# sb17v/GaussianK-SGD

Measured on AMD Instinct MI355X. Metric: images/sec (whole node) ResNet-50 k=0.1% at 1/2/4/8 MI355X; effective grad compression ratio, higher is better.
Workload: dtype fp32; 1 GPU; model=resnet50, global_batch=512, per_gpu_batch=512, image_size=224, parallelism=dp1, compressor=gaussian, buckets=1, threshold=524288000, planner=threshold, exchange=local, momentum_correction=True, hip_graph=False, f32_matmul=bf16x6

## Files before the change

### gaussiank_sgd_amd/ops/autotune.py

```python
from __future__ import annotations

import os
from typing import Callable, Dict, Iterable, List, Optional, Tuple

import torch

_TUNE = os.environ.get("GKSGD_GEMM_TUNE", "1") != "0"
_choices: Dict[tuple, tuple] = {}
_OWN = ("hip", "w3", "mat", "wino", "wx6")
_GK_MARGIN = float(os.environ.get("GKSGD_GK_MARGIN", "0.05"))
_timings: Dict[tuple, list] = {}
_NT_CFGS = [1, 2, 3, 4, 11, 13, 21, 22, 23, 24, 111, 113, 121, 122, 123, 124, 25, 26, 27, 125, 126, 127,
            211, 212, 213, 214, 221, 222, 223, 224]
NT_GRIDS = (0, 512, 1 << 20)
_TN_CFGS = [(c, s) for c in (1, 2, 3, 4, 5, 6, 7, 8, 21, 22, 23, 24, 27, 9, 29, 101, 121, 102, 122) for s in (0, 128)]
_NT_CFGS_F32 = [1, 2, 3, 4, 7, 11, 12, 13, 14, 21, 22, 23, 24, 101, 102, 103, 104, 201, 202, 203, 204,
                1001, 1002, 1003, 1004, 1005, 1006, 1007, 1021, 1022, 1101, 1102, 1103]
_TN_CFGS_F32 = [(c, s) for c in (1, 2, 3, 4, 5, 6, 7, 8, 9, 11, 12, 13, 14, 15, 16) for s in (0, 64)]
_TN_SMALL_M = 1 << 17
_TN_SMALL_F32 = [(c, s) for c in (4, 5, 11, 14, 15) for s in (16, 32, 128)]


X6 = 100000
_NT_CFGS_X6 = [c + X6 for c in (1, 2, 3, 4, 5, 6, 7, 12, 13, 101, 102, 103, 104, 105, 106, 107, 202, 203, 1001, 1002, 1003)]
_NT_CFGS_X62 = [2 * X6 + t for t in range(1, 8)] + [3 * X6 + t for t in range(1, 8)]
_F32MM = os.environ.get("GKSGD_F32_MATMUL", "bf16x6")


def set_f32_matmul(mode: str) -> str:
    global _F32MM
    if mode not in ("native", "bf16x6"):
        raise ValueError("f32 matmul mode must be 'native' or 'bf16x6', got %r" % (mode,))
# ... 156 lines not shown
```

### gaussiank_sgd_amd/ops/build.py

```python
from __future__ import annotations

import argparse
import concurrent.futures as cf
import hashlib
import os
import re
import shutil
import subprocess
import sys
import sysconfig
from pathlib import Path
from typing import List

PKG = Path(__file__).resolve().parents[1]
REPO = PKG.parent
CSRC = PKG / "ops" / "csrc"
BUILD = REPO / "build" / "gksgd_ext"
TARGET = PKG / "_C.so"
ASAN = os.environ.get("GKSGD_ASAN", "0") == "1"
if ASAN:
    BUILD = REPO / "build" / "gksgd_ext_asan"
    TARGET = REPO / "build" / "asan" / "_C.so"
SAN_HOST = ["-fsanitize=address", "-fsanitize=undefined"]
VARIANT = os.environ.get("GKSGD_VARIANT", "")
VARIANT_FLAGS = os.environ.get("GKSGD_VARIANT_FLAGS", "").split()
if VARIANT and not ASAN:
    BUILD = REPO / "build" / ("gksgd_ext_" + VARIANT)
    TARGET = REPO / "variants" / VARIANT / "_C.so"
ARCH = os.environ.get("GKSGD_OFFLOAD_ARCH", "gfx950")
ROCM = os.environ.get("ROCM_PATH", "/opt/rocm")

GEMM_UNIT_FAMILY = ["nt", "nt", "nt", "nt", "tn", "nt", "nt", "tn", "nt_x62", "tn_x62", "nt_x62"]
HIP_SOURCES = [
    "kernels/compress.hip",
    "kernels/quality.hip",
    "kernels/scatter.hip",
    "kernels/optim.hip",
    "kernels/bn_act.hip",
    "kernels/gemm.hip",
    *["kernels/gemm_inst_%s.hip#%d" % (f, u) for u, f in enumerate(GEMM_UNIT_FAMILY)],
    "kernels/ln.hip",
    "kernels/linear.hip",
    "kernels/lstm.hip",
    "kernels/stem.hip",
    "kernels/wgrad3.hip",
    "kernels/attn.hip",
    "kernels/attn_f32.hip",
    "kernels/embed.hip",
    "kernels/xent.hip",
    "kernels/winograd.hip",
    "kernels/wino_x6.hip",
    "kernels/stem_f32.hip",
    "kernels/prep.hip",
]
CXX_SOURCES = [
    "comm/rccl_engine.cpp",
    "bindings.cpp",
]
EXTRA_FLAGS = {"kernels/scatter.hip": ["-ffp-contract=off"],
               **{"kernels/gemm_inst_%s.hip" % f: ["-fno-slp-vectorize"] for f in set(GEMM_UNIT_FAMILY)}}


def _torch_dirs():
    import torch
    tdir = Path(torch.__file__).resolve().parent
    return tdir / "include", tdir / "include" / "torch" / "csrc" / "api" / "include", tdir / "lib"


def _hipcc() -> str:
    p = shutil.which("hipcc") or os.path.join(ROCM, "bin", "hipcc")
    return p


def _hip_flags() -> List[str]:
    san = []
    if ASAN:
        for f in SAN_HOST:
            san += ["-Xarch_host", f]
        san += ["-Xarch_host", "-fno-omit-frame-pointer"]
    return san + VARIANT_FLAGS + [
        "--offload-arch=" + ARCH,
        "-O3",
        "-fPIC",
# ... 131 lines not shown
```

### gaussiank_sgd_amd/ops/conv1x1.py

```python
from __future__ import annotations

import os
from itertools import product
from typing import Dict

import torch
import torch.nn as nn
import torch.nn.functional as F

from . import autotune
from . import load
from . import streams
from . import weight_prep
from .autotune import (X6, f32_matmul, load_choices, save_choices, set_f32_matmul,
                       tuned_choices, tuning_log)

_CL = torch.channels_last
_ENABLED = os.environ.get("GKSGD_FASTCONV", "1") != "0"
_BIAS_COLSUM = os.environ.get("GKSGD_CONV_BIAS_COLSUM", "1") != "0"
_WINO = os.environ.get("GKSGD_WINO", "1") != "0"
_FORCE = os.environ.get("GKSGD_CONV_FORCE", "")
_WINO_GRIDS = (0, 1 << 20)
_zeros: Dict[torch.device, torch.Tensor] = {}

# ... 286 lines not shown
    return ch is None or ch[0] == "hip"


def _dgrad_bn_ds(dy: torch.Tensor, w: torch.Tensor, x_shape, link, wp: bool = False) -> torch.Tensor:
    N, C, H, W, K, k, p, OH, OW = _geom(x_shape, w, 1)
    g = _g()
    M = N * H * W
    dt = dy.dtype
    dz = torch.empty(x_shape, dtype=dt, device=dy.device, memory_format=_CL)
    st = torch.empty(2, min(1280, (M + 63) // 64), C, dtype=torch.float32, device=dy.device)
    DY, DZ, H2 = _rows(dy), _rows(dz), _rows(link.h)
    D2, geo, mask = link.dy2c, list(link.geo), link.mask
    Wt = _lazy(lambda: weight_prep.transposed_1x1(w, wp))
    run = lambda c, mb: g.gemm_nt(DY, Wt(), DZ, c, mb, st, None, H2, D2, mask, bn_dy2_geo=geo)
    cands = autotune.hip_cands(run, product(autotune.nt_x62_cfgs(), autotune.NT_GRIDS))
    ch = autotune.pick(("dgrad_bn_ds", N, C, H, W, K) + autotune.dkey(dt), cands)
    rows = run(ch[1], ch[2])
    link.part = (st, int(rows))
    link.dz = dz
    link.dy2c = None
    return dz


def _bn_fusable(link, s: int, dgrad_key: tuple) -> bool:
    if link is None or s != 1 or not _link_on() or not link.ready():
        return False
    if link.h.dtype != dgrad_key_dtype(dgrad_key):
        return False
    ch = autotune.choice(dgrad_key)
    return ch is None or ch[0] in ("hip", "wino", "wx6")


def dgrad_key_dtype(key: tuple) -> torch.dtype:
    return torch.float32 if "f32" in key[8:] else torch.bfloat16


def _wgrad_key(x: torch.Tensor, w: torch.Tensor, s: int, lz=None) -> tuple:
    N, C, H, W, K, k, p, OH, OW = _geom(x.shape, w, s)
    wino = lz is None and _wino_ok(x.dtype, k, s, C, K) and C % 64 == 0 and _wino_shape_fits(N, H, W, C, K)
    return ("wgrad", N, C, H, W, K, k, s) + autotune.dkey(x.dtype) + (("lz",) if lz is not None else ()) + \
        (("wino",) if wino else ())


def _wgrad_into(dy: torch.Tensor, x: torch.Tensor, w: torch.Tensor, s: int, out_f32: torch.Tensor, lz=None,
                plink=None, side: bool = False) -> None:
    N, C, H, W, K, k, p, OH, OW = _geom(x.shape, w, s)
# ... 108 lines not shown
        gvb = getattr(bs0, "grad_view", None) if bs0 is not None else None
        bias_fork = fork and _FORK_BIAS and _BIAS_COLSUM and gvb is not None and gvb.is_contiguous() and \
            not getattr(bs0, "shared", False) and dy.is_contiguous(memory_format=_CL)

        def fork_wgrad():
            sink.check()
            if bias_fork:
                bs0.check()
            side = streams.fork(x.device)
            with torch.cuda.stream(side):
                _wgrad_into(dy, x, w, s, sink.grad_view, side=True)
                if bias_fork:
                    from .linear import bias_grad_acc_
                    bias_grad_acc_(gvb, _rows(dy))
            streams.hold(x.device, dy, x, w)
        if fork and not _WGRAD_AFTER:
            fork_wgrad()
        dx = None
        if ctx.needs_input_grad[0]:
            N, C, H, W = x.shape
            key = _dgrad_key(N, C, H, W, w.shape[0], w.shape[2], s, ctx.dt)
            prep, ctx.prep = ctx.prep, None
            with weight_prep.use(prep):
                if lz is None and _ds_compact_ok(ds_link, x, w, s, ctx.dt):
                    ds_link.dy2c = _dgrad_ds(dy, w, x.shape, wp=ctx.wp)
                    ds_link.geo = (H, W, dy.shape[2], dy.shape[3])
                elif link is not None and link.dy2c is not None:
                    if _ds_fusable(link, x, w, s, ctx.dt, key, lz):
                        dx = _dgrad_bn_ds(dy, w, x.shape, link, wp=ctx.wp)
                    else:
                        dx = _dgrad(dy, w, x.shape, s, lz, plink, wp=ctx.wp)
                elif _bn_fusable(link, s, key):
                    dx = _dgrad_bn(dy, w, x.shape, s, link, lz, plink, wp=ctx.wp)
                else:
                    dx = _dgrad(dy, w, x.shape, s, lz, plink, wp=ctx.wp)
        if fork and _WGRAD_AFTER:
            fork_wgrad()
        gparam = None
        if ctx.needs_input_grad[1] and not fork:
            if direct:
                sink.check()
                _wgrad_into(dy, x, w, s, sink.grad_view, lz, plink)
            else:
                out = torch.zeros(w.shape, dtype=torch.float32, device=x.device).contiguous(memory_format=_CL)
                _wgrad_into(dy, x, w, s, out, lz, plink)
                if sink is not None:
                    sink(out)
# ... 93 lines not shown
```

### gaussiank_sgd_amd/ops/csrc/bindings.cpp

```cpp
#include <ATen/ATen.h>
#include <c10/core/DeviceGuard.h>
#include <c10/hip/HIPStream.h>
#include <torch/custom_class.h>
#include <torch/library.h>

#include <cstring>
#include <vector>

#include "comm/rccl_engine.h"
#include "kernels/gemm_cfg.h"
#include "kernels/gk_kernels.h"

namespace {

hipStream_t cur_stream(const at::Tensor& t) {
  return c10::hip::getCurrentHIPStream(t.device().index()).stream();
}

void check_dev(const at::Tensor& t, const char* name) {
  TORCH_CHECK(t.is_cuda(), name, " must be a GPU tensor");
  TORCH_CHECK(t.is_contiguous(), name, " must be contiguous");
}

void check_f32(const at::Tensor& t, const char* name) {
// ... 1466 lines not shown
  if (k == 1) {
    const at::Tensor wt = w.reshape({K, C}).t().contiguous();
    const int r = gk::conv_nt_remap(dy.data_ptr(), K, zero.data_ptr(), (int)OHd, (int)OWd, (int)K, (int)OHd,
                                    (int)OWd, 1, 1, wt.data_ptr(), dx.data_ptr(), N * OHd * OWd, (int)C, (int)H, (int)W,
                                    0, 0, 1, f32, (int)cfg, (int)max_blocks, lz, st);
    TORCH_CHECK(r >= 0, "conv_dgrad_s2: the lazy operand's coefficient table does not fit this tile configuration");
    return;
  }
  const at::Tensor wt = w.permute({1, 2, 3, 0}).contiguous();
  for (int a = 0; a < 2; ++a) {
    for (int b = 0; b < 2; ++b) {
      const int64_t OHc = (H - a + 1) / 2, OWc = (W - b + 1) / 2;
      if (OHc <= 0 || OWc <= 0) continue;
      at::Tensor wc = a == 0 ? wt.slice(1, 1, 2) : wt.slice(1, 0, 3, 2).flip({1});
      wc = b == 0 ? wc.slice(2, 1, 2) : wc.slice(2, 0, 3, 2).flip({2});
      wc = wc.contiguous();
      const int r = gk::conv_nt_remap(dy.data_ptr(), K, zero.data_ptr(), (int)OHd, (int)OWd, (int)K, (int)OHc,
                                      (int)OWc, a == 0 ? 1 : 2, b == 0 ? 1 : 2, wc.data_ptr(), dx.data_ptr(),
                                      N * OHc * OWc, (int)C, (int)H, (int)W, a, b, 0, f32, (int)cfg, (int)max_blocks,
                                      lz, st);
      TORCH_CHECK(r >= 0, "conv_dgrad_s2: the lazy operand's coefficient table does not fit this tile configuration");
    }
  }
}

int64_t wgrad3_ws(int64_t N, int64_t H, int64_t W, int64_t C, int64_t K) {
  return gk::wgrad3_ws_floats((int)N, (int)H, (int)W, (int)C, (int)K);
}

void conv3_wgrad(at::Tensor dy, at::Tensor x, at::Tensor out, at::Tensor part, at::Tensor zero) {
  TORCH_CHECK(x.is_cuda() && x.scalar_type() == at::kBFloat16 && x.dim() == 4 &&
                  x.is_contiguous(at::MemoryFormat::ChannelsLast),
              "conv3_wgrad: x must be channels-last bf16 [N, C, H, W]");
  const int64_t N = x.size(0), C = x.size(1), H = x.size(2), W = x.size(3);
  TORCH_CHECK(dy.is_cuda() && dy.scalar_type() == at::kBFloat16 && dy.dim() == 4 && dy.size(0) == N &&
                  dy.size(2) == H && dy.size(3) == W && dy.is_contiguous(at::MemoryFormat::ChannelsLast),
              "conv3_wgrad: dy must be channels-last bf16 [N, K, H, W]");
  const int64_t K = dy.size(1);
  TORCH_CHECK(gk::wgrad3_supported((int)H, (int)W, (int)C, (int)K), "conv3_wgrad: unsupported shape");
  TORCH_CHECK(N * H * W < (int64_t(1) << 31), "conv3_wgrad: too many pixels");
  TORCH_CHECK(out.is_cuda() && out.scalar_type() == at::kFloat && out.dim() == 4 && out.size(0) == K &&
                  out.size(1) == C && out.size(2) == 3 && out.size(3) == 3,
              "conv3_wgrad: out must be fp32 [K, C, 3, 3]");
  TORCH_CHECK(part.is_cuda() && part.scalar_type() == at::kFloat && part.is_contiguous() &&
                  part.numel() >= wgrad3_ws(N, H, W, C, K),
              "conv3_wgrad: part must hold wgrad3_ws floats");
// ... 566 lines not shown
  m.def("stem_f32_supported(int H, int W) -> bool", [](int64_t H, int64_t W) { return gk::stem_f32_supported((int)H, (int)W); });
  m.def("stem_f32_fwd(Tensor x, Tensor w, Tensor(a!) y, Tensor(b!)? stats=None) -> int");
  m.def("stem_f32x6_wplanes() -> int", &stem_f32x6_wplanes);
  m.def("stem_f32x6_fwd(Tensor x, Tensor w, Tensor(a!) y, Tensor(b!)? stats, Tensor(c!) wp3) -> int");
  m.def("stem_f32_wgrad_ws(int N) -> int", &stem_f32_wgrad_ws);
  m.def("stem_f32_wgrad(Tensor x, Tensor dy, Tensor(a!) out, Tensor(b!) part, bool x6=False) -> ()");
  m.def("wgrad3_supported(int H, int W, int C, int K) -> bool", [](int64_t H, int64_t W, int64_t C, int64_t K) {
    return gk::wgrad3_supported((int)H, (int)W, (int)C, (int)K);
  });
  m.def("wgrad3_ws(int N, int H, int W, int C, int K) -> int", &wgrad3_ws);
  m.def("conv3_wgrad(Tensor dy, Tensor x, Tensor(a!) out, Tensor(b!) part, Tensor zero) -> ()");
  m.def("wino_weights(Tensor w, Tensor(a!) u, bool flip) -> ()");
  m.def("weight_prep(Tensor table, int ndesc, int total_blocks) -> ()");
  m.def("weight_prep_blocks(int kind, int R, int S) -> int", &weight_prep_blocks);
  m.def("wino_wgrad_ws(int N, int H, int W, int C, int K, int splits=0) -> int", &wino_wgrad_ws);
  m.def("wino_wgrad(Tensor x, Tensor dy, Tensor(a!) out, Tensor(b!) part, int splits=0) -> ()");
  m.def("wino_conv(Tensor x, Tensor u, Tensor(a!) y, int max_blocks=0, Tensor(b!)? stats=None, Tensor? bn_h=None, "
        "Tensor? bn_dy2=None, Tensor? bn_mask=None, int splits=1) -> int");
  m.def("wino_x6_weights(Tensor w, Tensor(a!) u3, bool flip) -> ()");
  m.def("wino_x6_conv(Tensor x, Tensor u3, Tensor(a!) y, int max_blocks=0, Tensor(b!)? stats=None, "
        "Tensor? bn_h=None, Tensor? bn_dy2=None, Tensor? bn_mask=None) -> int");
  m.def("conv_dgrad_s2(Tensor dy, Tensor w, Tensor(a!) dx, Tensor zero, int cfg=0, int max_blocks=0, "
        "Tensor? lz_x=None, Tensor? lz_coef=None, Tensor? lz_padz=None, Tensor? lz_padx=None) -> ()");
  m.def("bn_bwd_lazy_pre(Tensor x, Tensor part, int rows, Tensor? w, Tensor mean, Tensor invstd, "
        "Tensor(a!) dgamma, Tensor(b!) dbeta, Tensor(c!) coef, Tensor(d!) padz, Tensor(e!) padx, "
        "Tensor(f!)? gw_acc=None, Tensor(g!)? gb_acc=None) -> ()");
  m.def("bn_act_backward_lazy(Tensor dy, Tensor? dy2, Tensor? mask, Tensor x, Tensor(a!) dz, Tensor? w, "
        "Tensor mean, Tensor invstd, Tensor(b!) dgamma, Tensor(c!) dbeta, Tensor(d!) ws, bool relu, "
        "Tensor(e!) coef, Tensor(f!) padz, Tensor(g!) padx, Tensor(h!)? gw_acc=None, Tensor(i!)? gb_acc=None) -> ()");
  m.def("bn_lazy_apply(Tensor dz, Tensor x, Tensor(a!) dx, Tensor coef) -> ()");
  m.def("bn_stats_partials(Tensor x, Tensor(a!) ws) -> ()");
  m.def(
      "bn_act_backward_pre_dual(Tensor dz, Tensor x, Tensor(a!) dx, Tensor? w, Tensor mean, Tensor invstd, "
      "Tensor(b!) dgamma, Tensor(c!) dbeta, Tensor part, int rows, Tensor(d!)? gw_acc, Tensor(e!)? gb_acc, Tensor x2, "
      "Tensor(f!) dx2, Tensor? w2, Tensor mean2, Tensor invstd2, Tensor(g!) dgamma2, Tensor(h!) dbeta2, "
      "Tensor(i!) ws2, Tensor(j!)? gw2_acc, Tensor(k!)? gb2_acc) -> ()");
  m.def("bn_act_backward_pre(Tensor dz, Tensor x, Tensor(a!) dx, Tensor? w, Tensor mean, Tensor invstd, "
        "Tensor(b!) dgamma, Tensor(c!) dbeta, Tensor part, int rows, Tensor(d!)? gw_acc=None, "
        "Tensor(e!)? gb_acc=None, Tensor(f!)? fin=None) -> ()");
  m.def("bn_fin_state_bytes(int C) -> int", &bn_fin_state_bytes);
  m.def("attn_supported(int T, int D) -> bool",
        [](int64_t T, int64_t D) { return gk::attn_supported((int)T, (int)D); });
  m.def("attn_fwd(Tensor qkv, Tensor(a!) out, Tensor(b!) lse, int heads, float p, int seed, Tensor? seed_dev=None, "
        "Tensor? key_bits=None, Tensor(c!)? out_lo=None, bool causal=False) -> ()");
  m.def("attn_pack_key_mask(Tensor mask, Tensor(a!) bits) -> ()");
  m.def("attn_bwd(Tensor qkv, Tensor out, Tensor dout, Tensor lse, Tensor(a!) delta, Tensor(b!) dqkv, int heads, "
// ... 70 lines not shown
  m.impl("scatter_add_records", &scatter_add_records);
  m.impl("apply_records_sgd", &apply_records_sgd);
  m.impl("arena_digest", &arena_digest);
  m.impl("fill_zero", &fill_zero);
  m.impl("sign_bucket_compress", &sign_bucket_compress);
  m.impl("sign_bucket_decompress", &sign_bucket_decompress);
  m.impl("fused_sgd", &fused_sgd);
  m.impl("fused_adam", &fused_adam);
  m.impl("fused_lamb", &fused_lamb);
  m.impl("segmented_sumsq", &segmented_sumsq);
  m.impl("fused_lars", &fused_lars);
  m.impl("clip_grad_norm", &clip_grad_norm);
  m.impl("bn_act_forward", &bn_act_forward);
  m.impl("bn_act_finalize", &bn_act_finalize);
  m.impl("bn_act_backward", &bn_act_backward);
  m.impl("bn_act_backward_pre", &bn_act_backward_pre);
  m.impl("bn_act_backward_pre_dual", &bn_act_backward_pre_dual);
  m.impl("bn_bwd_lazy_pre", &bn_bwd_lazy_pre);
  m.impl("bn_act_backward_lazy", &bn_act_backward_lazy);
  m.impl("bn_lazy_apply", &bn_lazy_apply);
  m.impl("bn_stats_partials", &bn_stats_partials);
  m.impl("stem_pack", &stem_pack);
  m.impl("conv_dgrad_s2", &conv_dgrad_s2);
  m.impl("conv3_wgrad", &conv3_wgrad);
  m.impl("stem_fwd", &stem_fwd);
  m.impl("stem_wgrad", &stem_wgrad);
  m.impl("stem_f32_fwd", &stem_f32_fwd);
  m.impl("stem_f32x6_fwd", &stem_f32x6_fwd);
  m.impl("stem_f32_wgrad", &stem_f32_wgrad);
  m.impl("bn_relu_pool_forward", &bn_relu_pool_forward);
  m.impl("bn_relu_pool_backward", &bn_relu_pool_backward);
  m.impl("accum_grad", &accum_grad);
  m.impl("momentum_correct", &momentum_correct);
  m.impl("mask_records", &mask_records);
  m.impl("cast_bf16", &cast_bf16);
  m.impl("gemm_nt", &gemm_nt);
  m.impl("gemm_tn_acc", &gemm_tn_acc);
  m.impl("conv_nt", &conv_nt);
  m.impl("wino_weights", &wino_weights);
  m.impl("weight_prep", &weight_prep);
  m.impl("wino_conv", &wino_conv);
  m.impl("wino_x6_weights", &wino_x6_weights);
  m.impl("wino_x6_conv", &wino_x6_conv);
  m.impl("wino_wgrad", &wino_wgrad);
  m.impl("conv_tn_acc", &conv_tn_acc);
  m.impl("attn_fwd", &attn_fwd);
// ... 19 lines not shown
```

### gaussiank_sgd_amd/ops/csrc/kernels/gemm_nt_x62.h

```cpp
#pragma once

#include "gemm_common.h"

namespace gk {
namespace {

template <int WM, int WN>
struct X62Cfg {
  static constexpr int NW = WM * WN;
  static constexpr int THREADS = 64 * NW;
  static constexpr int BM = 64 * WM;
  static constexpr int BN = 64 * WN;
  static constexpr int PA = BM * 64;
  static constexpr int PB = BN * 64;
  static constexpr int STAGE = 3 * (PA + PB);
  static constexpr int LDS = 2 * STAGE;
  static constexpr int PRA = BM * 4 / THREADS;
  static constexpr int PRB = BN * 4 / THREADS;
  static_assert(PRA >= 1 && PRB >= 1 && (BM * 4) % THREADS == 0 && (BN * 4) % THREADS == 0, "pieces per thread");
  static_assert(LDS <= 160 * 1024, "LDS");
};

template <int WM, int WN, bool BNB, int NPF = 1, bool GATHER = false, bool P3 = false, bool D2C = false>
__global__ void __launch_bounds__(64 * WM * WN) __attribute__((amdgpu_waves_per_eu(1)))
gemm_nt_x62_kernel(const float* __restrict__ A, int64_t lda, const float* __restrict__ B, int64_t ldb,
                   float* __restrict__ C, int64_t ldc, int64_t M, int K, const float* __restrict__ bias,
                   float* __restrict__ stats, int64_t stats_ld, BnBwd bb, ConvGeo geo) {
  using Cfg = X62Cfg<WM, WN>;
  extern __shared__ __attribute__((aligned(16))) char smem[];
  int bx, by;
  xcd_remap2(bx, by);
  const int tid = threadIdx.x;
  const int lane = tid & 63;
  const int wave = __builtin_amdgcn_readfirstlane(tid >> 6);
  const int wm = wave / WN, wn = wave % WN;
  const int fr = lane & 15, fq = lane >> 4;
  const int n0 = by * Cfg::BN;
  const int Ntot = (int)gridDim.y * Cfg::BN;
  const int64_t mtiles = (M + Cfg::BM - 1) / Cfg::BM;
  const int nk = K / 32;
  const int64_t my_tiles = bx < mtiles ? (mtiles - 1 - bx) / gridDim.x + 1 : 0;
  const int T_ = (int)(my_tiles * nk);
  if (T_ == 0) {
    if (stats)
      for (int c = tid; c < Cfg::BN; c += Cfg::THREADS) {
        stats[(int64_t)bx * Ntot + n0 + c] = 0.f;
// ... 137 lines not shown
  for (int a = 0; a < 4; ++a)
#pragma unroll
    for (int b = 0; b < 4; ++b) acc[a][b] = f32x4{0.f, 0.f, 0.f, 0.f};
  float ssum[4][4], ssq[4][4], bia[BNB ? 1 : 4][4];
#pragma unroll
  for (int a = 0; a < 4; ++a)
#pragma unroll
    for (int b = 0; b < 4; ++b) {
      ssum[a][b] = ssq[a][b] = 0.f;
      if constexpr (!BNB) bia[a][b] = bias ? bias[n0 + wn * 64 + a * 16 + fq * 4 + b] : 0.f;
    }

  auto epilogue = [&](int64_t mt) __attribute__((always_inline)) {
    const int64_t mbase = mt * Cfg::BM;
    constexpr int EH = BNB ? 1 : 4;
#pragma unroll
    for (int ms = 0; ms < 4; ++ms) {
      const int64_t m = mbase + wm * 64 + ms * 16 + fr;
      const bool live = m < M;
#pragma unroll
      for (int nh = 0; nh < 4; nh += EH) {
      f32x4 ehv[EH], ed2[EH];
      uint32_t ebits[EH];
      if constexpr (BNB) {
#pragma unroll
        for (int e = 0; e < EH; ++e) {
          ehv[e] = ed2[e] = f32x4{0.f, 0.f, 0.f, 0.f};
          ebits[e] = 0u;
        }
        if (live) {
          int32_t d2row = -1;
          if constexpr (BNB && D2C) {
            const uint32_t mu = (uint32_t)m;
            const uint32_t img = (__umulhi(mu, bb.mg_hw) + mu) >> bb.sh_hw, rem = mu - img * (uint32_t)(bb.H * bb.W);
            const uint32_t ph = (__umulhi(rem, bb.mg_w) + rem) >> bb.sh_w, pw = rem - ph * (uint32_t)bb.W;
            if (((ph | pw) & 1u) == 0u) d2row = (int32_t)((img * (uint32_t)bb.OH + (ph >> 1)) * (uint32_t)bb.OW + (pw >> 1));
          }
#pragma unroll
          for (int e = 0; e < EH; ++e) {
            const int n = n0 + wn * 64 + (nh + e) * 16 + fq * 4;
            ehv[e] = *reinterpret_cast<const f32x4*>(static_cast<const float*>(bb.h) + m * ldc + n);
            if constexpr (D2C) {
              if (d2row >= 0)
                ed2[e] = *reinterpret_cast<const f32x4*>(static_cast<const float*>(bb.dy2) + (int64_t)d2row * ldc + n);
            } else {
              if (bb.dy2) ed2[e] = *reinterpret_cast<const f32x4*>(static_cast<const float*>(bb.dy2) + m * ldc + n);
            }
            ebits[e] = bb.mask ? (uint32_t)bb.mask[m * (Ntot >> 2) + (n >> 2)] : 0xfu;
          }
        }
      }
#pragma unroll
      for (int e = 0; e < EH; ++e) {
        const int ns = nh + e;
        const int n = n0 + wn * 64 + ns * 16 + fq * 4;
        f32x4 v = acc[ms][ns];
        acc[ms][ns] = f32x4{0.f, 0.f, 0.f, 0.f};
        if constexpr (!BNB) {
#pragma unroll
          for (int r = 0; r < 4; ++r) v[r] += bia[ns][r];
        }
        if constexpr (BNB) {
#pragma unroll
          for (int r = 0; r < 4; ++r) {
            const float dz = (ebits[e] >> r) & 1u ? v[r] + ed2[e][r] : 0.f;
            v[r] = dz;
            ssum[ns][r] += dz;
            ssq[ns][r] = fmaf(dz, ehv[e][r], ssq[ns][r]);
          }
        } else {
          if (stats && live) {
#pragma unroll
            for (int r = 0; r < 4; ++r) {
              ssum[ns][r] += v[r];
              ssq[ns][r] = fmaf(v[r], v[r], ssq[ns][r]);
            }
          }
        }
        if (live) *reinterpret_cast<f32x4*>(C + m * ldc + n) = v;
      }
      }
    }
  };

  using I0 = std::integral_constant<int, 0>;
  using I1 = std::integral_constant<int, (NPF > 1 ? 1 : 0)>;
  issue_loads(I0{});
  split_write(0, I0{});
  if (T_ > 1) issue_loads(I1{});
  if (NPF > 1 && T_ > 2) issue_loads(I0{});
  __syncthreads();
  int ks = 0;
  int64_t mt = bx;
  auto slice = [&](int t, auto PAR) __attribute__((always_inline)) {
    constexpr int par = decltype(PAR)::value;
    using SN = std::integral_constant<int, (NPF > 1 ? (par ^ 1) : 0)>;
    const int cur = par;
    const char* st = smem + cur * Cfg::STAGE;
    const char* pa = st;
    const char* pb = st + 3 * Cfg::PA;
    auto frag = [&](const char* plane, int row) __attribute__((always_inline)) -> bf16x8 {
      return *reinterpret_cast<const bf16x8*>(plane + row * 64 + ((fq ^ x62_swz(row)) << 4));
// ... 53 lines not shown
#pragma unroll
      for (int a = 0; a < 4; ++a)
#pragma unroll
        for (int b = 0; b < 4; ++b) {
          const int col = wn * 64 + a * 16 + fq * 4 + b;
          red[wm * Cfg::BN + col] = ssum[a][b];
          red[(WM + wm) * Cfg::BN + col] = ssq[a][b];
        }
    }
    __syncthreads();
    for (int c = tid; c < Cfg::BN; c += Cfg::THREADS) {
      float sa = 0.f, sb = 0.f;
#pragma unroll
      for (int w2 = 0; w2 < WM; ++w2) {
        sa += red[w2 * Cfg::BN + c];
        sb += red[(WM + w2) * Cfg::BN + c];
      }
      stats[(int64_t)bx * Ntot + n0 + c] = sa;
      stats[stats_ld + (int64_t)bx * Ntot + n0 + c] = sb;
    }
  }
}

template <int WM, int WN, bool BNB, int NPF, bool GATHER, bool P3 = false, bool D2C = false>
int launch_nt_x62(const float* A, int64_t lda, const float* B, int64_t ldb, float* C, int64_t ldc, int64_t M, int N,
                  int K, int max_blocks, const float* bias, float* stats, int64_t stats_ld, int stats_rows,
                  const BnBwd& bb, const ConvGeo& geo, hipStream_t stream) {
  using Cfg = X62Cfg<WM, WN>;
  const int ntiles = N / Cfg::BN;
  const int64_t mtiles = (M + Cfg::BM - 1) / Cfg::BM;
  const int per_cu = (160 * 1024) / Cfg::LDS > 0 ? (160 * 1024) / Cfg::LDS : 1;
  int64_t gx = ((int64_t)256 * per_cu + ntiles - 1) / ntiles;
  if (max_blocks > 0) gx = max_blocks;
  if (gx < 1) gx = 1;
  if (gx > mtiles) gx = mtiles;
  if (stats && gx > stats_rows) gx = stats_rows;
  static bool attr = [] {
    return hipFuncSetAttribute(reinterpret_cast<const void*>(&gemm_nt_x62_kernel<WM, WN, BNB, NPF, GATHER, P3, D2C>),
                               hipFuncAttributeMaxDynamicSharedMemorySize, 160 * 1024) == hipSuccess;
  }();
  (void)attr;
  hipLaunchKernelGGL((gemm_nt_x62_kernel<WM, WN, BNB, NPF, GATHER, P3, D2C>), dim3((unsigned)gx, (unsigned)ntiles), dim3(Cfg::THREADS),
                     Cfg::LDS, stream, A, lda, B, ldb, C, ldc, M, K, bias, stats, stats_ld, bb, geo);
  return (int)gx;
}

template <bool GATHER>
int nt_x62_dispatch(const float* A, int64_t lda, const float* B, int64_t ldb, float* C, int64_t ldc, int64_t M,
                    int N, int K, const cfg::NtWord& w, int max_blocks, const float* bias, float* stats,
                    int64_t stats_ld, int stats_rows, const BnBwd& bb, const ConvGeo& geo, hipStream_t stream) {
  const cfg::X62NtSel s = cfg::nt_x62_select(w, N, geo.b3 != nullptr, bb.h != nullptr);
#define GK_X62L(WM_, WN_, BNB_, P3_, D2C_)                                                                   \
  launch_nt_x62<WM_, WN_, BNB_, 1, GATHER, P3_, D2C_>(A, lda, B, ldb, C, ldc, M, N, K, max_blocks, bias, stats, \
                                                      stats_ld, stats_rows, bb, geo, stream)
#define GK_X62N(WM_, WN_, P3_)                                             \
  do {                                                                     \
    if constexpr (!GATHER)                                                 \
      if (s.bnb && bb.OW > 0) return GK_X62L(WM_, WN_, true, P3_, true);   \
    return s.bnb ? GK_X62L(WM_, WN_, true, P3_, false) : GK_X62L(WM_, WN_, false, P3_, false); \
  } while (0)
#define GK_X62(WM_, WN_)               \
  case cfg::x62_key(WM_, WN_):         \
    if (s.p3) GK_X62N(WM_, WN_, true); \
    GK_X62N(WM_, WN_, false)
  switch (cfg::x62_key(s.wm, s.wn)) {
    GK_X62(2, 4);
    GK_X62(4, 2);
    GK_X62(1, 4);
    GK_X62(4, 1);
    GK_X62(1, 2);
    GK_X62(2, 1);
    GK_X62(2, 2);
  }
#undef GK_X62
#undef GK_X62N
#undef GK_X62L
  return cfg::kDoesNotFit;
// ... 5 lines not shown
```

### gaussiank_sgd_amd/ops/csrc/kernels/gk_kernels.h

```cpp
#pragma once

#include <hip/hip_runtime.h>
#include <stddef.h>
#include <stdint.h>

namespace gk {

enum Mode : int {
  kModeGaussian = 0,
  kModeRedSync = 1,
  kModeRedSyncTrim = 2,
  kModeTopK = 3,
  kModeRandomK = 4,
  kModeThreshold = 5,
  kModeDGC = 6,
  kModeGaussianCal = 7,
};

constexpr int kCalFallback = 16;
constexpr int kOverflowExact = 17;

constexpr int kMaxCand = 16;
constexpr int kRecHdr = 4;
constexpr int kMaxCountBlocks = 1024;
// ... 252 lines not shown
};
struct LazyArgs {
  const void* x;
  const float* coef;
  const void* padz;
  const void* padx;
  int C;
};
int gemm_nt(const void* A, int64_t lda, const void* B, int64_t ldb, void* C, int64_t ldc, int64_t M, int N, int K,
            bool f32, int cfg, int max_blocks, float* stats, int stats_rows, const float* bias, const BnBwdArgs* bn,
            const LazyArgs* lazy, hipStream_t stream, float* splitk_ws = nullptr, const void* b3 = nullptr);
int splitk_reduce(const float* ws, int S, int64_t M, int N, float* C, int64_t ldc, const float* bias, float* stats,
                  int stats_rows, const BnBwdArgs* bn, hipStream_t stream);
int gemm_tn_acc(const void* G, int64_t ldg, const void* X, int64_t ldx, float* W, int64_t ldw, int64_t M, int N,
                 int K, bool f32, int cfg, int splits, const LazyArgs* lazy, hipStream_t stream);
int conv_nt(const void* X, const void* zero, int H, int W, int C, int OH, int OW, int S, int P, int KH, int KW,
            const void* B, void* Y, int64_t M, int N, bool f32, int cfg, int max_blocks, float* stats, int stats_rows,
            const float* bias, const BnBwdArgs* bn, const LazyArgs* lazy, hipStream_t stream,
            float* splitk_ws = nullptr, const void* b3 = nullptr);
void split3_rows(const float* src, int64_t ld, void* dst, int64_t R, int S, hipStream_t stream);
int conv_nt_remap(const void* X, int64_t ldx, const void* zero, int H, int W, int C, int OH, int OW, int KH, int KW,
                  const void* B, void* Y, int64_t M, int N, int RH, int RW, int RA, int RB, int RZ, bool f32, int cfg,
                  int max_blocks, const LazyArgs* lazy, hipStream_t stream);
int conv_tn_acc(const void* G, const void* X, const void* zero, int H, int W, int C, int OH, int OW, int S, int P,
                 int KH, int KW, float* Wout, int64_t M, int N, bool f32, int cfg, int splits, const LazyArgs* lazy,
                 hipStream_t stream);
bool stem_f32_supported(int H, int W);
int stem_f32_wgrad_blocks(int N);
int stem_f32x6_wplanes();
int stem_f32x6_forward(const float* x, int N, int H, int W, const float* w, int64_t s0, int64_t s1, int64_t s2,
                       int64_t s3, uint16_t* wp3, float* y, float* stats, int stats_rows, hipStream_t stream);
int stem_f32_forward(const float* x, int N, int H, int W, const float* w, int64_t s0, int64_t s1, int64_t s2,
                     int64_t s3, float* y, float* stats, int stats_rows, hipStream_t stream);
void stem_f32_wgrad(const float* x, const float* dy, int N, int H, int W, float* part, float* out, int64_t s0,
                    int64_t s1, int64_t s2, int64_t s3, bool x6, hipStream_t stream);
void wino_weights(const float* w, float* u, int Co, int Ci, int flip, hipStream_t stream);
enum PrepKind : int32_t { kPrepWino = 0, kPrepWinoFlip = 1, kPrepT32 = 2, kPrepT16 = 3, kPrepWinoX6 = 4,
                          kPrepWinoX6Flip = 5 };
struct PrepDesc {
  const void* src;
  void* dst;
  int64_t ld_in, ld_out;
  int64_t block_begin;
  int32_t kind, R, S, tiles_s;
};
static_assert(sizeof(PrepDesc) == 56, "PrepDesc layout is packed by ops/weight_prep.py");
// ... 95 lines not shown
```

### gaussiank_sgd_amd/ops/weight_prep.py

```python
from __future__ import annotations

import contextlib
import os
import struct
import threading
from typing import Callable, Dict, List, Optional, Tuple

import torch

KIND_WINO, KIND_WINO_FLIP, KIND_T32, KIND_T16, KIND_WINO_X6, KIND_WINO_X6_FLIP = 0, 1, 2, 3, 4, 5
_DESC = struct.Struct("<QQqqqiiii")
_MAX_DESCS = 512
_tls = threading.local()
ENABLED = os.environ.get("GKSGD_WEIGHT_PREP", "1") != "0"


def _ops():
    return torch.ops.gksgd


class _Entry:
    __slots__ = ("src", "dst", "descs", "ready")

    def __init__(self, src: torch.Tensor, dst: torch.Tensor, descs: List[tuple]):
# ... 146 lines not shown


def flipped_3x3(w: torch.Tensor, persistent: bool) -> torch.Tensor:
    K, C = w.shape[0], w.shape[1]

    def make():
        return torch.empty((C, K, 3, 3), dtype=w.dtype, device=w.device, memory_format=torch.channels_last)

    def fill(out):
        out.copy_(w.flip(2, 3).transpose(0, 1))
    p = current()
    if p is None or not persistent or w.dtype not in (torch.float32, torch.bfloat16) or \
            not w.is_contiguous(memory_format=torch.channels_last):
        out = make()
        fill(out)
        return out
    kind = KIND_T32 if w.dtype == torch.float32 else KIND_T16
    es = w.element_size()

    def descs(out):
        return [(kind, w.data_ptr() + (8 - t) * C * es, out.data_ptr() + t * K * es, 9 * C, 9 * K, K, C)
                for t in range(9)]
    return p.acquire(_key("f3", w), w, make, descs, fill)
```

Baseline: 5221 images/s.

## Add bf16x6 stride-2 3x3 dgrad via sub-pixel class decomposition with fused BN backward

Adds a stride-2 3x3 data-gradient path that splits the transposed convolution into four output-parity classes. Each class is a dense implicit GEMM run through the register-staged bf16x6 NT kernel, writing into the strided dx positions through a new S2C epilogue remap. This avoids the zero-stuffed or gather-heavy work of the generic s2 dgrad. An optional fused BN-backward epilogue gathers stats partials in the same pass. The autotuner can still fall back to the existing path, now tagged 'base' and treated as an in-house candidate, at the cost of extra tuning time and a per-call weight reorder when the weights are not persistent.

```diff
diff --git a/gaussiank_sgd_amd/ops/autotune.py b/gaussiank_sgd_amd/ops/autotune.py
--- a/gaussiank_sgd_amd/ops/autotune.py
+++ b/gaussiank_sgd_amd/ops/autotune.py
@@ -7,7 +7,7 @@
 
 _TUNE = os.environ.get("GKSGD_GEMM_TUNE", "1") != "0"
 _choices: Dict[tuple, tuple] = {}
-_OWN = ("hip", "w3", "mat", "wino", "wx6")
+_OWN = ("hip", "w3", "mat", "wino", "wx6", "base")
 _GK_MARGIN = float(os.environ.get("GKSGD_GK_MARGIN", "0.05"))
 _timings: Dict[tuple, list] = {}
 _NT_CFGS = [1, 2, 3, 4, 11, 13, 21, 22, 23, 24, 111, 113, 121, 122, 123, 124, 25, 26, 27, 125, 126, 127,
diff --git a/gaussiank_sgd_amd/ops/build.py b/gaussiank_sgd_amd/ops/build.py
--- a/gaussiank_sgd_amd/ops/build.py
+++ b/gaussiank_sgd_amd/ops/build.py
@@ -38,6 +38,7 @@
     "kernels/optim.hip",
     "kernels/bn_act.hip",
     "kernels/gemm.hip",
+    "kernels/dgrad_s2_x62.hip",
     *["kernels/gemm_inst_%s.hip#%d" % (f, u) for u, f in enumerate(GEMM_UNIT_FAMILY)],
     "kernels/ln.hip",
     "kernels/linear.hip",
@@ -58,7 +59,8 @@
     "bindings.cpp",
 ]
 EXTRA_FLAGS = {"kernels/scatter.hip": ["-ffp-contract=off"],
-               **{"kernels/gemm_inst_%s.hip" % f: ["-fno-slp-vectorize"] for f in set(GEMM_UNIT_FAMILY)}}
+               **{"kernels/gemm_inst_%s.hip" % f: ["-fno-slp-vectorize"] for f in set(GEMM_UNIT_FAMILY)},
+               "kernels/dgrad_s2_x62.hip": ["-fno-slp-vectorize"]}
 
 
 def _torch_dirs():
diff --git a/gaussiank_sgd_amd/ops/conv1x1.py b/gaussiank_sgd_amd/ops/conv1x1.py
--- a/gaussiank_sgd_amd/ops/conv1x1.py
+++ b/gaussiank_sgd_amd/ops/conv1x1.py
@@ -332,6 +332,73 @@
     return dz
 
 
+_S2X = os.environ.get("GKSGD_DGRAD_S2_X62", "1") != "0"
+_BASE = ("base", 0, 0)
+
+
+def _s2x_ok(w: torch.Tensor, s: int, dt: torch.dtype, lz) -> bool:
+    return _S2X and s == 2 and w.shape[2] == 3 and dt == torch.float32 and lz is None and \
+        f32_matmul() == "bf16x6"
+
+
+def _dgrad_s2x(dy: torch.Tensor, w: torch.Tensor, x_shape, wp: bool = False) -> torch.Tensor:
+    N, C, H, W, K, k, p, OH, OW = _geom(x_shape, w, 2)
+    g = _g()
+    dt = dy.dtype
+    dx = torch.empty(x_shape, dtype=dt, device=dy.device, memory_format=_CL)
+    z = _zero(dy.device)
+    wc = _lazy(lambda: weight_prep.s2_class_weights(w, wp))
+    run = lambda c, mb: g.conv_dgrad_s2_x62(dy, wc(), dx, z, c, mb)
+    cands = autotune.hip_cands(run, product(autotune.nt_x62_cfgs(), autotune.NT_GRIDS))
+    cands.append((_BASE, lambda: _dgrad(dy, w, x_shape, 2, wp=wp)))
+    ch = autotune.pick(("dgrad_s2x", N, C, H, W, K) + autotune.dkey(dt), cands)
+    if ch[0] == "base":
+        return _dgrad(dy, w, x_shape, 2, wp=wp)
+    run(ch[1], ch[2])
+    return dx
+
+
+def _dgrad_bn_s2(dy: torch.Tensor, w: torch.Tensor, x_shape, link, wp: bool = False) -> torch.Tensor:
+    N, C, H, W, K, k, p, OH, OW = _geom(x_shape, w, 2)
+    g = _g()
+    dt = dy.dtype
+    dz = torch.empty(x_shape, dtype=dt, device=dy.device, memory_format=_CL)
+    st = torch.empty(2, 4 * min(512, (N * ((H + 1) // 2) * ((W + 1) // 2) + 63) // 64), C, dtype=torch.float32,
+                     device=dy.device)
+    h, mask = link.h, link.mask
+    z = _zero(dy.device)
+    wc = _lazy(lambda: weight_prep.s2_class_weights(w, wp))
+    run = lambda c, mb: g.conv_dgrad_s2_x62(dy, wc(), dz, z, c, mb, st, h, mask)
+    key = ("dgrad_bn", N, C, H, W, K, k, 2, False) + autotune.dkey(dt)
+    cands = autotune.hip_cands(run, product(autotune.nt_x62_cfgs(), autotune.NT_GRIDS))
+    if autotune.choice(key) is None:
+        mean, invstd = torch.zeros(C, device=dy.device), torch.ones(C, device=dy.device)
+        gs = torch.empty(2, C, dtype=torch.float32, device=dy.device)
+        dxs = torch.empty_like(h, memory_format=_CL)
+        ws = torch.empty(int(g.bn_workspace_floats(N * H * W, C, h.element_size())), dtype=torch.float32,
+                         device=dy.device)
+
+        def fused(fn):
+            g.bn_act_backward_pre(dz, h, dxs, None, mean, invstd, gs[0], gs[1], st, int(fn()))
+
+        def base():
+            g.bn_act_backward(_dgrad(dy, w, x_shape, 2, wp=wp), mask, h, dxs, None, None, mean, invstd, gs[0], gs[1],
+                              ws, mask is not None)
+        cands = [(tag, (lambda fn=fn: fused(fn))) for tag, fn in cands] + [(_BASE, base)]
+    ch = autotune.pick(key, cands)
+    if ch[0] == "base":
+        return _dgrad(dy, w, x_shape, 2, wp=wp)
+    rows = run(ch[1], ch[2])
+    link.part = (st, int(rows))
+    link.dz = dz
+    return dz
+
+
+def _bn_s2_fusable(link, x: torch.Tensor, dt: torch.dtype) -> bool:
+    return link is not None and _link_on() and link.ready() and link.dy2 is None and link.dy2c is None and \
+        link.h.dtype == dt and link.h.shape == x.shape
+
+
 def _bn_fusable(link, s: int, dgrad_key: tuple) -> bool:
     if link is None or s != 1 or not _link_on() or not link.ready():
         return False
@@ -486,7 +553,12 @@
             key = _dgrad_key(N, C, H, W, w.shape[0], w.shape[2], s, ctx.dt)
             prep, ctx.prep = ctx.prep, None
             with weight_prep.use(prep):
-                if lz is None and _ds_compact_ok(ds_link, x, w, s, ctx.dt):
+                if _s2x_ok(w, s, ctx.dt, lz):
+                    if _bn_s2_fusable(link, x, ctx.dt):
+                        dx = _dgrad_bn_s2(dy, w, x.shape, link, wp=ctx.wp)
+                    else:
+                        dx = _dgrad_s2x(dy, w, x.shape, wp=ctx.wp)
+                elif lz is None and _ds_compact_ok(ds_link, x, w, s, ctx.dt):
                     ds_link.dy2c = _dgrad_ds(dy, w, x.shape, wp=ctx.wp)
                     ds_link.geo = (H, W, dy.shape[2], dy.shape[3])
                 elif link is not None and link.dy2c is not None:
diff --git a/gaussiank_sgd_amd/ops/csrc/bindings.cpp b/gaussiank_sgd_amd/ops/csrc/bindings.cpp
--- a/gaussiank_sgd_amd/ops/csrc/bindings.cpp
+++ b/gaussiank_sgd_amd/ops/csrc/bindings.cpp
@@ -1512,6 +1512,53 @@
       TORCH_CHECK(r >= 0, "conv_dgrad_s2: the lazy operand's coefficient table does not fit this tile configuration");
     }
   }
+}
+
+int64_t conv_dgrad_s2_x62(at::Tensor dy, at::Tensor wcls, at::Tensor dx, at::Tensor zero, int64_t cfg,
+                          int64_t max_blocks, c10::optional<at::Tensor> stats, c10::optional<at::Tensor> bn_h,
+                          c10::optional<at::Tensor> bn_mask, c10::optional<at::Tensor> lz_x) {
+  TORCH_CHECK(!lz_x.has_value() || !lz_x->defined(), "conv_dgrad_s2_x62: no lazy operand (conv_dgrad_s2 takes one)");
+  TORCH_CHECK(dy.is_cuda() && dy.scalar_type() == at::kFloat && dy.dim() == 4 &&
+                  dy.is_contiguous(at::MemoryFormat::ChannelsLast),
+              "conv_dgrad_s2_x62: dy must be channels-last fp32");
+  TORCH_CHECK(dx.is_cuda() && dx.scalar_type() == at::kFloat && dx.dim() == 4 && dx.size(0) == dy.size(0) &&
+                  dx.is_contiguous(at::MemoryFormat::ChannelsLast),
+              "conv_dgrad_s2_x62: dx must be channels-last fp32 [N, C, H, W]");
+  const int64_t N = dy.size(0), K = dy.size(1), OH = dy.size(2), OW = dy.size(3);
+  const int64_t C = dx.size(1), H = dx.size(2), W = dx.size(3);
+  TORCH_CHECK((H - 1) / 2 + 1 == OH && (W - 1) / 2 + 1 == OW, "conv_dgrad_s2_x62: shape mismatch");
+  TORCH_CHECK(K % 64 == 0 && C % 64 == 0 && dy.numel() > 0, "conv_dgrad_s2_x62: channels must be multiples of 64");
+  TORCH_CHECK(wcls.is_cuda() && wcls.scalar_type() == at::kFloat && wcls.is_contiguous() && wcls.numel() == 9 * C * K &&
+                  reinterpret_cast<uintptr_t>(wcls.data_ptr()) % 16 == 0,
+              "conv_dgrad_s2_x62: wcls must hold the four class matrices, 9 * C * K contiguous fp32");
+  check_zero(zero);
+  TORCH_CHECK(dy.numel() < (int64_t(1) << 31) && N * H * W < (int64_t(1) << 31), "conv_dgrad_s2_x62: too many elements");
+  const gk::cfg::NtWord word = gk::cfg::NtWord::decode((int)cfg);
+  TORCH_CHECK(word.family >= 2 && word.planes <= 1,
+              "conv_dgrad_s2_x62: register-staged bf16x6 configurations only (cfg digit 200000 / 300000)");
+  int rows = 0;
+  float* sp = stats_ptr(stats, C, &rows);
+  gk::BnBwdArgs bn{};
+  const bool has_bn = bn_bwd_args(bn_h, c10::nullopt, bn_mask, N * H * W, C, C, sp != nullptr, at::kFloat, &bn);
+  TORCH_CHECK(!has_bn || rows >= 4, "conv_dgrad_s2_x62: the BN-backward epilogue needs >= 4 partial rows");
+  TORCH_CHECK(has_bn || sp == nullptr, "conv_dgrad_s2_x62: stats come with the BN-backward epilogue only");
+  c10::DeviceGuard guard(dy.device());
+  const hipStream_t st = cur_stream(dy);
+  at::Tensor b3;
+  if (word.family == 3) {
+    b3 = at::empty({27 * C * K}, wcls.options().dtype(at::kBFloat16));
+    for (int cls = 0; cls < 4; ++cls) {
+      const int64_t off = gk::s2_class_offset(cls) * C * K, taps = (1 + (cls >> 1)) * (1 + (cls & 1));
+      gk::split3_rows(wcls.data_ptr<float>() + off, taps * K, static_cast<at::BFloat16*>(b3.data_ptr()) + 3 * off, C,
+                      (int)(taps * K), st);
+    }
+  }
+  const int r = gk::conv_dgrad_s2_x62(dy.data_ptr<float>(), zero.data_ptr(), (int)N, (int)OH, (int)OW, (int)K,
+                                      wcls.data_ptr<float>(), b3.defined() ? b3.data_ptr() : nullptr,
+                                      dx.data_ptr<float>(), (int)C, (int)H, (int)W, (int)cfg, (int)max_blocks, sp, rows,
+                                      has_bn ? &bn : nullptr, st);
+  TORCH_CHECK(r >= 0, "conv_dgrad_s2_x62: refused (", r, "): fp32, cfg family 2 / 3, 32-bit offsets");
+  return r;
 }
 
 int64_t wgrad3_ws(int64_t N, int64_t H, int64_t W, int64_t C, int64_t K) {
@@ -2124,6 +2171,8 @@
         "Tensor? bn_h=None, Tensor? bn_dy2=None, Tensor? bn_mask=None) -> int");
   m.def("conv_dgrad_s2(Tensor dy, Tensor w, Tensor(a!) dx, Tensor zero, int cfg=0, int max_blocks=0, "
         "Tensor? lz_x=None, Tensor? lz_coef=None, Tensor? lz_padz=None, Tensor? lz_padx=None) -> ()");
+  m.def("conv_dgrad_s2_x62(Tensor dy, Tensor wcls, Tensor(a!) dx, Tensor zero, int cfg, int max_blocks=0, "
+        "Tensor(b!)? stats=None, Tensor? bn_h=None, Tensor? bn_mask=None, Tensor? lz_x=None) -> int");
   m.def("bn_bwd_lazy_pre(Tensor x, Tensor part, int rows, Tensor? w, Tensor mean, Tensor invstd, "
         "Tensor(a!) dgamma, Tensor(b!) dbeta, Tensor(c!) coef, Tensor(d!) padz, Tensor(e!) padx, "
         "Tensor(f!)? gw_acc=None, Tensor(g!)? gb_acc=None) -> ()");
@@ -2240,6 +2289,7 @@
   m.impl("bn_stats_partials", &bn_stats_partials);
   m.impl("stem_pack", &stem_pack);
   m.impl("conv_dgrad_s2", &conv_dgrad_s2);
+  m.impl("conv_dgrad_s2_x62", &conv_dgrad_s2_x62);
   m.impl("conv3_wgrad", &conv3_wgrad);
   m.impl("stem_fwd", &stem_fwd);
   m.impl("stem_wgrad", &stem_wgrad);
diff --git a/gaussiank_sgd_amd/ops/csrc/kernels/dgrad_s2_x62.hip b/gaussiank_sgd_amd/ops/csrc/kernels/dgrad_s2_x62.hip
--- /dev/null
+++ b/gaussiank_sgd_amd/ops/csrc/kernels/dgrad_s2_x62.hip
@@ -0,0 +1,37 @@
+#include "gemm_nt_x62.h"
+
+namespace gk {
+
+int conv_dgrad_s2_x62(const float* dy, const void* zero, int N, int OH, int OW, int K, const float* wcls,
+                      const void* wcls3, float* dx, int C, int H, int W, int cfg, int max_blocks, float* stats,
+                      int stats_rows, const BnBwdArgs* bn, hipStream_t stream) {
+  const cfg::NtWord w = cfg::NtWord::decode(cfg);
+  if (w.family < 2 || (w.family == 3) != (wcls3 != nullptr)) return cfg::kRowGemmsOnly;
+  if (K % 32 != 0 || C % 64 != 0 || (int64_t)N * OH * OW * K >= ((int64_t)1 << 31) ||
+      (int64_t)N * H * W >= ((int64_t)1 << 31))
+    return cfg::kRowGemmsOnly;
+  if (bn && (bn->dy2 || !stats || stats_rows < 4)) return cfg::kDoesNotFit;
+  if (!bn) stats = nullptr;
+  const int64_t CK = (int64_t)C * K;
+  int rows = 0;
+  for (int cls = 0; cls < 4; ++cls) {
+    const int a = cls >> 1, b = cls & 1;
+    const int OHc = (H - a + 1) / 2, OWc = (W - b + 1) / 2;
+    if (OHc <= 0 || OWc <= 0) continue;
+    const int KHc = 1 + a, KWc = 1 + b;
+    const int Kc = KHc * KWc * K;
+    ConvGeo g{zero, OH, OW, K, OHc, OWc, 1, 0, KWc, nullptr, H, W, a, b, 0};
+    if (wcls3) g.b3 = static_cast<const uint16_t*>(wcls3) + 3 * s2_class_offset(cls) * CK;
+    BnBwd bb = bn ? BnBwd{bn->h, nullptr, bn->mask} : BnBwd{};
+    magic_u32((uint32_t)(OHc * OWc), &bb.mg_hw, &bb.sh_hw);
+    magic_u32((uint32_t)OWc, &bb.mg_w, &bb.sh_w);
+    const int r = nt_x62_dispatch<true, true>(dy, K, wcls + s2_class_offset(cls) * CK, Kc, dx, C, (int64_t)N * OHc * OWc,
+                                              C, Kc, w, max_blocks, nullptr, stats ? stats + (int64_t)rows * C : nullptr,
+                                              (int64_t)stats_rows * C, stats_rows / 4, bb, g, stream);
+    if (r < 0) return r;
+    rows += r;
+  }
+  return rows;
+}
+
+}
diff --git a/gaussiank_sgd_amd/ops/csrc/kernels/gemm_nt_x62.h b/gaussiank_sgd_amd/ops/csrc/kernels/gemm_nt_x62.h
--- a/gaussiank_sgd_amd/ops/csrc/kernels/gemm_nt_x62.h
+++ b/gaussiank_sgd_amd/ops/csrc/kernels/gemm_nt_x62.h
@@ -21,7 +21,8 @@
   static_assert(LDS <= 160 * 1024, "LDS");
 };
 
-template <int WM, int WN, bool BNB, int NPF = 1, bool GATHER = false, bool P3 = false, bool D2C = false>
+template <int WM, int WN, bool BNB, int NPF = 1, bool GATHER = false, bool P3 = false, bool D2C = false,
+          bool S2C = false>
 __global__ void __launch_bounds__(64 * WM * WN) __attribute__((amdgpu_waves_per_eu(1)))
 gemm_nt_x62_kernel(const float* __restrict__ A, int64_t lda, const float* __restrict__ B, int64_t ldb,
                    float* __restrict__ C, int64_t ldc, int64_t M, int K, const float* __restrict__ bias,
@@ -205,6 +206,14 @@
       for (int nh = 0; nh < 4; nh += EH) {
       f32x4 ehv[EH], ed2[EH];
       uint32_t ebits[EH];
+      int64_t om = m;
+      if constexpr (S2C) {
+        const uint32_t mu = live ? (uint32_t)m : 0u;
+        const uint32_t img = (__umulhi(mu, bb.mg_hw) + mu) >> bb.sh_hw, rem = mu - img * (uint32_t)(geo.OH * geo.OW);
+        const uint32_t oh = (__umulhi(rem, bb.mg_w) + rem) >> bb.sh_w, ow = rem - oh * (uint32_t)geo.OW;
+        om = (int64_t)((img * (uint32_t)geo.RH + 2u * oh + (uint32_t)geo.RA) * (uint32_t)geo.RW + 2u * ow +
+                       (uint32_t)geo.RB);
+      }
       if constexpr (BNB) {
 #pragma unroll
         for (int e = 0; e < EH; ++e) {
@@ -222,14 +231,15 @@
 #pragma unroll
           for (int e = 0; e < EH; ++e) {
             const int n = n0 + wn * 64 + (nh + e) * 16 + fq * 4;
-            ehv[e] = *reinterpret_cast<const f32x4*>(static_cast<const float*>(bb.h) + m * ldc + n);
-            if constexpr (D2C) {
+            ehv[e] = *reinterpret_cast<const f32x4*>(static_cast<const float*>(bb.h) + om * ldc + n);
+            if constexpr (S2C) {
+            } else if constexpr (D2C) {
               if (d2row >= 0)
                 ed2[e] = *reinterpret_cast<const f32x4*>(static_cast<const float*>(bb.dy2) + (int64_t)d2row * ldc + n);
             } else {
               if (bb.dy2) ed2[e] = *reinterpret_cast<const f32x4*>(static_cast<const float*>(bb.dy2) + m * ldc + n);
             }
-            ebits[e] = bb.mask ? (uint32_t)bb.mask[m * (Ntot >> 2) + (n >> 2)] : 0xfu;
+            ebits[e] = bb.mask ? (uint32_t)bb.mask[om * (Ntot >> 2) + (n >> 2)] : 0xfu;
           }
         }
       }
@@ -260,7 +270,7 @@
             }
           }
         }
-        if (live) *reinterpret_cast<f32x4*>(C + m * ldc + n) = v;
+        if (live) *reinterpret_cast<f32x4*>(C + om * ldc + n) = v;
       }
       }
     }
@@ -360,7 +370,7 @@
   }
 }
 
-template <int WM, int WN, bool BNB, int NPF, bool GATHER, bool P3 = false, bool D2C = false>
+template <int WM, int WN, bool BNB, int NPF, bool GATHER, bool P3 = false, bool D2C = false, bool S2C = false>
 int launch_nt_x62(const float* A, int64_t lda, const float* B, int64_t ldb, float* C, int64_t ldc, int64_t M, int N,
                   int K, int max_blocks, const float* bias, float* stats, int64_t stats_ld, int stats_rows,
                   const BnBwd& bb, const ConvGeo& geo, hipStream_t stream) {
@@ -374,23 +384,23 @@
   if (gx > mtiles) gx = mtiles;
   if (stats && gx > stats_rows) gx = stats_rows;
   static bool attr = [] {
-    return hipFuncSetAttribute(reinterpret_cast<const void*>(&gemm_nt_x62_kernel<WM, WN, BNB, NPF, GATHER, P3, D2C>),
+    return hipFuncSetAttribute(reinterpret_cast<const void*>(&gemm_nt_x62_kernel<WM, WN, BNB, NPF, GATHER, P3, D2C, S2C>),
                                hipFuncAttributeMaxDynamicSharedMemorySize, 160 * 1024) == hipSuccess;
   }();
   (void)attr;
-  hipLaunchKernelGGL((gemm_nt_x62_kernel<WM, WN, BNB, NPF, GATHER, P3, D2C>), dim3((unsigned)gx, (unsigned)ntiles), dim3(Cfg::THREADS),
+  hipLaunchKernelGGL((gemm_nt_x62_kernel<WM, WN, BNB, NPF, GATHER, P3, D2C, S2C>), dim3((unsigned)gx, (unsigned)ntiles), dim3(Cfg::THREADS),
                      Cfg::LDS, stream, A, lda, B, ldb, C, ldc, M, K, bias, stats, stats_ld, bb, geo);
   return (int)gx;
 }
 
-template <bool GATHER>
+template <bool GATHER, bool S2C = false>
 int nt_x62_dispatch(const float* A, int64_t lda, const float* B, int64_t ldb, float* C, int64_t ldc, int64_t M,
                     int N, int K, const cfg::NtWord& w, int max_blocks, const float* bias, float* stats,
                     int64_t stats_ld, int stats_rows, const BnBwd& bb, const ConvGeo& geo, hipStream_t stream) {
   const cfg::X62NtSel s = cfg::nt_x62_select(w, N, geo.b3 != nullptr, bb.h != nullptr);
 #define GK_X62L(WM_, WN_, BNB_, P3_, D2C_)                                                                   \
-  launch_nt_x62<WM_, WN_, BNB_, 1, GATHER, P3_, D2C_>(A, lda, B, ldb, C, ldc, M, N, K, max_blocks, bias, stats, \
-                                                      stats_ld, stats_rows, bb, geo, stream)
+  launch_nt_x62<WM_, WN_, BNB_, 1, GATHER, P3_, D2C_, S2C>(A, lda, B, ldb, C, ldc, M, N, K, max_blocks, bias, stats, \
+                                                           stats_ld, stats_rows, bb, geo, stream)
 #define GK_X62N(WM_, WN_, P3_)                                             \
   do {                                                                     \
     if constexpr (!GATHER)                                                 \
diff --git a/gaussiank_sgd_amd/ops/csrc/kernels/gk_kernels.h b/gaussiank_sgd_amd/ops/csrc/kernels/gk_kernels.h
--- a/gaussiank_sgd_amd/ops/csrc/kernels/gk_kernels.h
+++ b/gaussiank_sgd_amd/ops/csrc/kernels/gk_kernels.h
@@ -298,6 +298,10 @@
 int conv_nt_remap(const void* X, int64_t ldx, const void* zero, int H, int W, int C, int OH, int OW, int KH, int KW,
                   const void* B, void* Y, int64_t M, int N, int RH, int RW, int RA, int RB, int RZ, bool f32, int cfg,
                   int max_blocks, const LazyArgs* lazy, hipStream_t stream);
+constexpr int s2_class_offset(int cls) { return cls == 0 ? 0 : (cls == 1 ? 1 : (cls == 2 ? 3 : 5)); }
+int conv_dgrad_s2_x62(const float* dy, const void* zero, int N, int OH, int OW, int K, const float* wcls,
+                      const void* wcls3, float* dx, int C, int H, int W, int cfg, int max_blocks, float* stats,
+                      int stats_rows, const BnBwdArgs* bn, hipStream_t stream);
 int conv_tn_acc(const void* G, const void* X, const void* zero, int H, int W, int C, int OH, int OW, int S, int P,
                  int KH, int KW, float* Wout, int64_t M, int N, bool f32, int cfg, int splits, const LazyArgs* lazy,
                  hipStream_t stream);
diff --git a/gaussiank_sgd_amd/ops/weight_prep.py b/gaussiank_sgd_amd/ops/weight_prep.py
--- a/gaussiank_sgd_amd/ops/weight_prep.py
+++ b/gaussiank_sgd_amd/ops/weight_prep.py
@@ -192,3 +192,41 @@
         return [(kind, w.data_ptr() + (8 - t) * C * es, out.data_ptr() + t * K * es, 9 * C, 9 * K, K, C)
                 for t in range(9)]
     return p.acquire(_key("f3", w), w, make, descs, fill)
+
+
+S2_TAPS = ((1,), (2, 0))
+S2_CLASS_OFFSET = (0, 1, 3, 5)
+
+
+def s2_class_weights(w: torch.Tensor, persistent: bool) -> torch.Tensor:
+    K, C = w.shape[0], w.shape[1]
+
+    def make():
+        return torch.empty(9 * C * K, dtype=w.dtype, device=w.device)
+
+    def fill(out):
+        wt = w.permute(1, 2, 3, 0)
+        for cls in range(4):
+            a, b = divmod(cls, 2)
+            wc = wt[:, 1:2] if a == 0 else wt[:, 0:3:2].flip(1)
+            wc = wc[:, :, 1:2] if b == 0 else wc[:, :, 0:3:2].flip(2)
+            o = S2_CLASS_OFFSET[cls] * C * K
+            out[o:o + wc.numel()].view(wc.shape).copy_(wc)
+    p = current()
+    if p is None or not persistent or w.dtype != torch.float32 or \
+            not w.is_contiguous(memory_format=torch.channels_last):
+        out = make()
+        fill(out)
+        return out
+    es = w.element_size()
+
+    def descs(out):
+        d = []
+        for cls in range(4):
+            th, tw = S2_TAPS[cls // 2], S2_TAPS[cls % 2]
+            taps = len(th) * len(tw)
+            for j, (kh, kw) in enumerate((kh, kw) for kh in th for kw in tw):
+                d.append((KIND_T32, w.data_ptr() + (kh * 3 + kw) * C * es,
+                          out.data_ptr() + (S2_CLASS_OFFSET[cls] * C * K + j * K) * es, 9 * C, taps * K, K, C))
+        return d
+    return p.acquire(_key("s2c", w), w, make, descs, fill)
```

Result: no change. 5238 images/s, median of 6 (+0.3%).
